# AIM-SE/AC-TSR

Hardware: AMD Instinct MI355X
Metric: user-sequences/sec fwd+bwd, AC-SASRec L=50 d=64, 1/2/4/8 MI355X (higher is better)
Workload: dtype f32; 1 GPU; ACSASRec full training step (spatial + adversarial calibrators, BASELINE configs[2]), synthetic 100000-item catalogue, B=512/GPU L=50 d=64 h=2 2 layers inner=256, CE loss, two-pass backward + Adam; global_batch=512, seq_len=50, hidden=64, heads=2, parallelism=dp1, launch=hipGraph replay per step, backward=two walks (reference protocol, trainer.py:672-686)

## Files before the change

### ac_tsr_amd/_lib.py

```python
from __future__ import annotations

import ctypes as C
import os
import subprocess

_HERE = os.path.dirname(os.path.abspath(__file__))
CSRC = os.path.join(_HERE, "csrc")
LIB_PATH = os.environ.get("ACATTN_LIB") or os.path.join(CSRC, "libacattn.so")
HEADER_PATH = os.path.join(os.path.dirname(_HERE), "include", "acattn.h")

ABI_VERSION = 34
MAX_MASKS = 8
NSTAT = 8
MASK_STRUCTURED, MASK_DENSE_LL, MASK_DENSE_L = 0, 1, 2
COMBINE = {"fixed": 0, "gate": 1, "annealing": 2}
RICH = {"none": 0, "fixed": 1, "trainable": 2}
RNG_EXPLICIT, RNG_COUNTER = 0, 1
FWD_AUTO, FWD_STREAM, FWD_STAGED, FWD_GENERAL = 0, 1, 2, 3
BWD_AUTO, BWD_STREAM, BWD_ROW = 0, 1, 2

_f = C.c_void_p


class Problem(C.Structure):
# ... 157 lines not shown
    "acattn_split_weights_many": (C.c_int, [C.POINTER(SplitLayer), C.c_int32, C.c_void_p]),
    "acattn_projections_split_bytes": (C.c_int64, [C.c_int32, C.c_int32]),
    "acattn_adam_step": (C.c_int, [C.POINTER(AdamGroup), C.c_double, C.c_double, C.c_double, C.c_double, C.c_double, _f,
                                   C.c_void_p]),
    "acattn_adam_step_cached": (C.c_int, [C.POINTER(AdamGroup), C.c_double, C.c_double, C.c_double, C.c_double, C.c_double, _f,
                                          C.c_void_p, C.c_void_p]),
    "acattn_select_adam_grid": (C.c_int, [C.c_int]),
    "acattn_dense_ce_fwd": (C.c_int, [_f, C.c_int64, C.c_int64, _f, _f, _f, C.c_void_p]),
    "acattn_dense_ce_bwd": (C.c_int, [_f, _f, _f, _f, C.c_int64, C.c_int64, _f, C.c_void_p]),
    "acattn_step_inputs": (C.c_int, [C.POINTER(C.c_void_p), C.POINTER(C.c_void_p), C.POINTER(C.c_int64), C.c_int32, C.c_void_p,
                                     C.c_void_p, C.c_void_p, C.c_int32, C.c_void_p]),
    "acattn_sum_rows": (C.c_int, [_f, _f, C.c_int32, C.c_int32, C.c_int32, C.c_void_p]),
    "acattn_sum_rows_pair": (C.c_int, [_f, _f, C.c_int32, C.c_int32, C.c_int32, _f, _f, C.c_int32, C.c_int32, C.c_int32, C.c_void_p]),
    "acattn_mask_penalty_fwd": (C.c_int, [_f, C.c_int64, _f, _f, C.c_void_p]),
    "acattn_mask_penalty_partial": (C.c_int, [_f, C.c_int64, _f, C.c_void_p]),
    "acattn_mask_penalty_partial_multi": (C.c_int, [C.c_void_p, C.c_int32, C.c_int64, _f, C.c_void_p]),
    "acattn_mask_penalty_bwd_scaled_multi": (C.c_int, [C.c_void_p, _f, _f, C.c_float, C.c_int64, C.c_void_p, C.c_int32,
                                                       C.c_void_p]),
    "acattn_attacked_loss_finish": (C.c_int, [_f, C.c_int32, _f, C.c_int32, C.c_int64, C.c_float, _f, _f, C.c_int32,
                                              C.c_void_p]),
    "acattn_mask_penalty_rows": (C.c_int, [_f, C.c_int32, C.c_int32, C.c_int32, _f, C.c_void_p]),
    "acattn_attacked_loss_finish_rows": (C.c_int, [_f, C.c_int32, C.c_void_p, C.c_int32, C.c_int32, C.c_float, _f, _f, C.c_int32,
                                                  C.c_void_p]),
    "acattn_attacked_loss_finish_rows_pair": (C.c_int, [_f, C.c_int32, C.c_void_p, C.c_int32, C.c_int32, C.c_float, _f, _f,
                                                       C.c_int32, _f, C.c_int32, _f, C.c_void_p]),
    "acattn_mask_penalty_drows": (C.c_int, [_f, _f, C.c_float, C.c_int32, C.c_void_p, C.c_int32, C.c_void_p]),
    "acattn_mask_penalty_drows_dir": (C.c_int, [_f, _f, C.c_float, C.c_int32, C.c_void_p, C.c_int32, _f, _f, C.c_int32, C.c_void_p]),
    "acattn_mask_penalty_bwd_scaled": (C.c_int, [_f, _f, _f, C.c_float, C.c_int64, _f, C.c_void_p]),
    "acattn_mask_penalty_bwd": (C.c_int, [_f, _f, _f, C.c_int64, _f, C.c_void_p]),
    "acattn_linear_wgrad_workspace_bytes": (C.c_int64, [C.c_int64, C.c_int32, C.c_int32]),
    "acattn_linear_wgrad_grouped": (C.c_int, [C.c_void_p, C.c_void_p, C.c_void_p, C.c_void_p, C.c_void_p, C.c_void_p,
                                               C.c_int32, C.c_int64, _f, C.c_void_p]),
    "acattn_linear_wgrad": (C.c_int, [_f, _f, C.c_int64, C.c_int32, C.c_int32, _f, _f, _f, C.c_void_p]),
    "acattn_linear_wgrad_grouped_partial": (C.c_int, [C.c_void_p, C.c_void_p, C.c_void_p, C.c_void_p, C.c_void_p, C.c_int32,
                                                       C.c_int64, C.c_void_p, C.c_void_p, C.c_void_p, C.c_void_p, C.c_void_p]),
    "acattn_linear_wgrad_reduce_many": (C.c_int, [C.c_void_p, C.c_void_p, C.c_void_p, C.c_void_p, C.c_void_p, C.c_void_p,
                                                   C.c_void_p, C.c_int32, C.c_void_p, C.c_void_p, C.c_void_p, C.c_void_p,
                                                   C.c_int32, C.c_void_p]),
    "acattn_select_forward_kernel": (C.c_int, [C.c_int]),
    "acattn_select_backward_kernel": (C.c_int, [C.c_int]),
    "acattn_calibrated_attention_bwd_workspace_bytes": (C.c_int64, [C.POINTER(Problem)]),
    "acattn_rng_materialize": (C.c_int, [C.c_int32, C.c_int32, C.c_int32, C.c_uint64, C.c_float, _f, _f, _f, _f,
                                         C.c_void_p]),
}

_lib = None


class AcattnError(RuntimeError):
    pass


def build(verbose: bool = False) -> str:
    jobs = str(min(8, os.cpu_count() or 1))
    res = subprocess.run(["make", "-C", CSRC, "-j", jobs], capture_output=not verbose, text=True)
    if res.returncode != 0:
        raise AcattnError("building libacattn.so failed:\n" + (res.stdout or "") + (res.stderr or ""))
    return LIB_PATH


def load() -> C.CDLL:
    global _lib
    if _lib is not None:
        return _lib
    if not os.path.exists(LIB_PATH):
        raise AcattnError(
# ... 24 lines not shown
```

### ac_tsr_amd/csrc/acattn_api.hip

```cpp
#include <stdint.h>
#include <stdio.h>
#include <string.h>

#include <algorithm>

#include "acattn_common.h"

namespace {
thread_local char g_err[256] = "";

int fail(const char* msg) {
  snprintf(g_err, sizeof(g_err), "%s", msg);
  return -1;
}

int check_problem(const acattn_problem* p) {
  if (!p) return fail("problem is NULL");
  if (p->B < 1 || p->L < 1 || p->H < 1 || p->n_heads < 1) return fail("B, L, H, n_heads must be positive");
  if (p->H % p->n_heads != 0)
    return fail("The hidden size is not a multiple of the number of attention heads");
  const int dh = p->H / p->n_heads;
  if (dh != 16 && dh != 32 && dh != 64 && dh != 128) return fail("unsupported head size: dh must be 16, 32, 64 or 128");
  if (p->L > 208) return fail("unsupported sequence length: L must be <= 208");
  if (!p->q || !p->k || !p->v) return fail("q, k, v must be non-NULL");
// ... 585 lines not shown
  if (rc > 0) snprintf(g_err, sizeof(g_err), "HIP launch failed: %s", hipGetErrorString((hipError_t)rc));
  return rc;
}

int acattn_adam_step_cached(const acattn_adam_group* g, double lr, double beta1, double beta2, double eps, double weight_decay,
                            int32_t* done, void* cache, void* stream) {
  if (!g || !done || !cache) return fail("group, done and cache must be non-NULL");
  if (((uintptr_t)cache & 15) != 0) return fail("cache must be 16-byte aligned");
  if (g->n_tensors < 1 || g->n_tensors > ACATTN_ADAM_MAX_TENSORS) return fail("1 <= n_tensors <= ACATTN_ADAM_MAX_TENSORS");
  int64_t trips = 0;
  for (int t = 0; t < g->n_tensors; ++t) {
    if (!g->param[t] || !g->grad[t] || !g->exp_avg[t] || !g->exp_avg_sq[t] || !g->step[t])
      return fail("param, grad, exp_avg, exp_avg_sq and step of every tensor must be non-NULL");
    if (g->numel[t] < 1) return fail("numel must be positive");
    trips += (g->numel[t] + 1023) / 1024;
  }
  if (trips >= (1ll << 30)) return fail("too many elements for one launch");
  if (!(beta1 >= 0 && beta1 < 1 && beta2 >= 0 && beta2 < 1)) return fail("betas must lie in [0, 1)");
  const int rc = acattn_launch_adam_step_cached(*g, lr, beta1, beta2, eps, weight_decay, done, cache, (hipStream_t)stream);
  if (rc > 0) snprintf(g_err, sizeof(g_err), "HIP launch failed: %s", hipGetErrorString((hipError_t)rc));
  return rc;
}

int acattn_select_adam_grid(int workgroups) {
  if (workgroups < 0 || workgroups > (1 << 20)) return fail("workgroups: 0 (by the device's compute units) or a positive count");
  return acattn_select_adam_grid_choice(workgroups);
}

int64_t acattn_linear_wgrad_workspace_bytes(int64_t M, int32_t K, int32_t N) {
  if (M < 1 || K < 1 || N < 1) return fail("M, K, N must be positive");
  return acattn_linear_wgrad_ws_bytes(M, K, N);
}

int acattn_linear_wgrad_grouped(const float* const* x, const float* const* dy, const int32_t* K, const int32_t* N,
                                float* const* dw, float* const* db, int32_t n_items, int64_t M, void* workspace,
                                void* stream) {
  if (!x || !dy || !K || !N || !dw || !db || !workspace) return fail("x, dy, K, N, dw, db and workspace must be non-NULL");
  if (n_items < 1 || n_items > ACATTN_WGRAD_MAX_GROUP) return fail("n_items must lie in [1, ACATTN_WGRAD_MAX_GROUP]");
  if (M < 1) return fail("M must be positive");
  for (int i = 0; i < n_items; ++i) {
    if (!x[i] || !dy[i] || !dw[i]) return fail("every item needs x, dy and dw");
    if (K[i] < 1 || N[i] < 1) return fail("K and N must be positive");
    if (M * (int64_t)std::max(K[i], N[i]) >= (1LL << 40)) return fail("matrix too large");
  }
  const int rc = acattn_launch_linear_wgrad(x, dy, (const int*)K, (const int*)N, dw, db, n_items, M, workspace,
                                            (hipStream_t)stream);
  if (rc > 0) snprintf(g_err, sizeof(g_err), "HIP launch failed: %s", hipGetErrorString((hipError_t)rc));
  return rc;
}

int acattn_linear_wgrad_grouped_partial(const float* const* x, const float* const* dy, const int32_t* K, const int32_t* N,
                                        const int32_t* want_bias, int32_t n_items, int64_t M, void* workspace, int32_t* n_partials,
                                        int64_t* w_offset, int64_t* b_offset, void* stream) {
  if (!x || !dy || !K || !N || !want_bias || !workspace || !n_partials || !w_offset || !b_offset)
    return fail("x, dy, K, N, want_bias, workspace, n_partials, w_offset and b_offset must be non-NULL");
  if (n_items < 1 || n_items > ACATTN_WGRAD_MAX_GROUP) return fail("n_items must lie in [1, ACATTN_WGRAD_MAX_GROUP]");
  if (M < 1) return fail("M must be positive");
  float* dw[ACATTN_WGRAD_MAX_GROUP];
  float* db[ACATTN_WGRAD_MAX_GROUP];
  for (int i = 0; i < n_items; ++i) {
    if (!x[i] || !dy[i]) return fail("every item needs x and dy");
    if (K[i] < 1 || N[i] < 1) return fail("K and N must be positive");
    if (M * (int64_t)std::max(K[i], N[i]) >= (1LL << 40)) return fail("matrix too large");
    dw[i] = nullptr;
    db[i] = want_bias[i] ? (float*)workspace : nullptr;
  }
  int P = 0;
  long long wo[ACATTN_WGRAD_MAX_GROUP], bo[ACATTN_WGRAD_MAX_GROUP];
  const int rc = acattn_launch_linear_wgrad(x, dy, (const int*)K, (const int*)N, dw, db, n_items, M, workspace,
                                            (hipStream_t)stream, &P, wo, bo);
  if (rc > 0) snprintf(g_err, sizeof(g_err), "HIP launch failed: %s", hipGetErrorString((hipError_t)rc));
  *n_partials = P;
  for (int i = 0; i < n_items; ++i) {
    w_offset[i] = wo[i];
    b_offset[i] = bo[i];
  }
  return rc;
}

int acattn_linear_wgrad_reduce_many(const float* const* part_w, const float* const* part_b, const int32_t* K, const int32_t* N,
                                    const int32_t* n_partials, float* const* dw, float* const* db, int32_t n_items,
// ... 28 lines not shown
```

### ac_tsr_amd/csrc/acattn_common.h

```cpp
#pragma once
#include <hip/hip_runtime.h>
#include <stdint.h>

#include <type_traits>

#include "acattn.h"

typedef float f4 __attribute__((ext_vector_type(4)));
typedef float f4u __attribute__((ext_vector_type(4), aligned(4)));

#define ACATTN_NEG_INF (-__builtin_inff())
#define ACATTN_MASK_FILL (-10000.0f)
#define ACATTN_LOG_EPS (1e-24f)

__device__ __forceinline__ float quad_sum(float x) {
  auto r = __builtin_amdgcn_permlane16_swap(__float_as_uint(x), __float_as_uint(x), false, false);
  x = __uint_as_float(r[0]) + __uint_as_float(r[1]);
  auto s = __builtin_amdgcn_permlane32_swap(__float_as_uint(x), __float_as_uint(x), false, false);
  return __uint_as_float(s[0]) + __uint_as_float(s[1]);
}

__device__ __forceinline__ float quad_max(float x) {
  auto r = __builtin_amdgcn_permlane16_swap(__float_as_uint(x), __float_as_uint(x), false, false);
  x = fmaxf(__uint_as_float(r[0]), __uint_as_float(r[1]));
// ... 245 lines not shown
int acattn_launch_ce_fwd(const acattn_ce_problem& p, void* ws, float* lse, float* row_loss, hipStream_t stream);
int acattn_launch_ce_fwd_dir(const acattn_ce_problem& p, void* ws, float* lse, float* row_loss, float* dir,
                             hipStream_t stream);
int acattn_launch_ce_bwd(const acattn_ce_problem& p, const float* lse, const float* coef, void* ws, float* d_out,
                         float* d_table, hipStream_t stream);
int acattn_launch_ln_fwd(const acattn_ln_problem& p, float* y, float* stats, hipStream_t stream);
int acattn_launch_ln_bwd(const acattn_ln_problem& p, const float* dy, const float* stats, float* dz, float* dres,
                         float* dgb_part, hipStream_t stream);
int acattn_launch_sum_rows(const float* x, float* out, int batch, int R, int C, hipStream_t stream);
int acattn_launch_sum_rows_pair(const float* x1, float* out1, int batch1, int R1, int C1, const float* x2, float* out2,
                                int batch2, int R2, int C2, hipStream_t stream);
void acattn_set_error(const char* msg);
bool acattn_proj_supported(int H, int G);
int64_t acattn_proj_bwd_ws_bytes(const acattn_proj_problem& p);
int acattn_launch_proj_fwd(const acattn_proj_problem& p, const acattn_proj_out& o, hipStream_t stream);
int64_t acattn_proj_split_bytes(int H, int G);
bool acattn_proj_qkv_supported(int H);
int acattn_launch_proj_qkv_fwd(const acattn_proj_problem& p, const acattn_proj_out& o, hipStream_t stream);
int acattn_launch_proj_bwd(const acattn_proj_problem& p, const acattn_proj_bwd_io& io, hipStream_t stream);
bool acattn_tail_supported(int H, int I);
int acattn_tail_bwd_partial_rows(int rows);
int acattn_tail_bwd_partial_rows_h(int rows, int H);
int64_t acattn_tail_bwd_ws_bytes(int H, int I);
int acattn_select_tail_nb(int nb);
int64_t acattn_tail_split_bytes(int H, int I, int rows);
int acattn_launch_tail_split(const acattn_tail_problem& p, void* planes, hipStream_t stream);
int acattn_launch_split_many(const acattn_split_layer* layers, int n_layers, hipStream_t stream);
int acattn_launch_tail_fwd(const acattn_tail_problem& p, const acattn_tail_saved& s, hipStream_t stream);
int acattn_launch_tail_bwd(const acattn_tail_problem& p, const acattn_tail_saved& s, const acattn_tail_bwd_io& io,
                           hipStream_t stream);
int64_t acattn_linear_wgrad_ws_bytes(int64_t M, int K, int N);
int acattn_launch_linear_wgrad(const float* const* x, const float* const* dy, const int* K, const int* N,
                               float* const* dw, float* const* db, int n_items, int64_t M, void* ws, hipStream_t stream,
                               int* P_out = nullptr, long long* w_off_out = nullptr, long long* b_off_out = nullptr);
int acattn_launch_linear_wgrad_reduce_many(const float* const* part_w, const float* const* part_b, const int* K, const int* N,
                                           const int* P, float* const* dw, float* const* db, int n_items,
                                           const float* const* sr_x, float* const* sr_out, const int* sr_R, const int* sr_C,
                                           int n_sr, hipStream_t stream);
int acattn_launch_embed_fwd(const acattn_embed_problem& p, float* y, float* stats, hipStream_t stream);
int acattn_launch_embed_bwd(const acattn_embed_problem& p, const float* dy, const float* stats, int64_t padding_idx,
                            float* d_table, float* d_pos_part, float* dgb_part, hipStream_t stream);
int acattn_launch_penalty_fwd(const float* m, int64_t n, float* ws, float* norm, hipStream_t stream);
int acattn_launch_penalty_partial(const float* m, int64_t n, float* part, hipStream_t stream);
void acattn_penalty_written_set(bool v);
bool acattn_penalty_written();
int acattn_launch_penalty_rows(const float* m, int B, int nh, int L, float* pen, hipStream_t stream);
int acattn_launch_attacked_loss_finish_rows(const float* row_loss, int B, const float* const* pen, int n_masks, int count,
                                            float weight, float* out, float* scale_buf, int n_scale, hipStream_t stream,
                                            const float* row_loss_c = nullptr, int B_c = 0, float* mean_c = nullptr);
int acattn_launch_penalty_drows(const float* norms, const float* d_loss, float scale, int count, float* const* d_pen,
                                int n_masks, hipStream_t stream, const float* dir = nullptr, float* d_out = nullptr, int n_dir = 0);
int acattn_launch_attacked_loss_finish(const float* row_loss, int B, const float* part, int n_masks, int64_t mask_numel,
                                       float weight, float* out, float* scale_buf, int n_scale, hipStream_t stream);
int acattn_launch_penalty_bwd_scaled(const float* m, const float* norm, const float* d_loss, float scale, int64_t n,
                                     float* d_m, hipStream_t stream);
int acattn_launch_penalty_bwd(const float* m, const float* norm, const float* d_norm, int64_t n, float* d_m,
                              hipStream_t stream);
int acattn_launch_zero(float* p, size_t n, hipStream_t stream);
int64_t acattn_ce6_rows_bytes(const acattn_ce_problem& p);
int acattn_launch_ce6_sweep(const acattn_ce_problem& p, const float* lse, const float* coef, float* slab, float* d_table,
                            float2* part, void* rows_ws, int n_wg, int n_left, bool dir, hipStream_t stream);
int acattn_launch_ce6_onehot_reduce(const acattn_ce_problem& p, const float* coef, const float* slab, int n_slabs, float* d_out,
                                    float* d_table, hipStream_t stream);
int acattn_launch_ce6_fwd_sweep(const acattn_ce_problem& p, float2* part, void* rows_ws, int n_wg, int n_left, hipStream_t stream);
int acattn_launch_ce6_pair_sweep(const acattn_ce_problem& pa, const acattn_ce_problem& pc, float* slab, float2* part_a,
                                 void* rows_a, float2* part_c, void* rows_c, int n_wg, int n_left, hipStream_t stream);
int64_t acattn_ce_pair_ws_bytes(const acattn_ce_problem& pa, const acattn_ce_problem& pc);
// ... 19 lines not shown
```

### ac_tsr_amd/csrc/acattn_linear.hip

```cpp
#include <stdlib.h>

#include <algorithm>

#include "acattn_common.h"
#include "acattn_sumrows.h"

namespace {

constexpr int kRegs = 64;

struct WgradGroup {
  const float* x[ACATTN_WGRAD_MAX_GROUP];
  const float* dy[ACATTN_WGRAD_MAX_GROUP];
  float* dw[ACATTN_WGRAD_MAX_GROUP];
  float* db[ACATTN_WGRAD_MAX_GROUP];
  int K[ACATTN_WGRAD_MAX_GROUP];
  int N[ACATTN_WGRAD_MAX_GROUP];
  long long w_off[ACATTN_WGRAD_MAX_GROUP];
  long long b_off[ACATTN_WGRAD_MAX_GROUP];
};

__device__ __forceinline__ f4 load_rows4(const float* base, int64_t row, int64_t M, int ld, int col, int ncols) {
  f4 v = {0.f, 0.f, 0.f, 0.f};
  if (row < M) {
    const float* p = base + row * ld + col;
    if (col + 3 < ncols) {
      v = *(const f4u*)p;
    } else {
#pragma unroll
      for (int e = 0; e < 4; ++e)
        if (col + e < ncols) v[e] = p[e];
    }
  }
  return v;
}

template <int UNROLL>
__global__ void __launch_bounds__(256, 2) wgrad_partial_kernel(const WgradGroup G, const int64_t M,
                                                             float* __restrict__ ws) {
  const int it = blockIdx.z;
  const int K = G.K[it], N = G.N[it];
  const int KB = (K + 63) >> 6, NB = (N + 63) >> 6;
  if ((int)blockIdx.y >= KB * NB) return;
  const float* __restrict__ x = G.x[it];
  const float* __restrict__ dy = G.dy[it];
  float* part_w = ws + G.w_off[it];
  float* part_b = G.db[it] ? ws + G.b_off[it] : nullptr;
  const int lane = threadIdx.x & 63, wave = threadIdx.x >> 6;
  const int c = lane & 15, g = lane >> 4;
  const int blk = blockIdx.y, nb = blk / KB, kb = blk - nb * KB;
  const int P = gridDim.x;
  const int ncol = nb * 64 + 4 * c, kcol = kb * 64 + 4 * c;

  f4 acc[4][4];
#pragma unroll
  for (int a = 0; a < 4; ++a)
#pragma unroll
    for (int b = 0; b < 4; ++b) acc[a][b] = f4{0.f, 0.f, 0.f, 0.f};
  f4 bsum = {0.f, 0.f, 0.f, 0.f};

  const int64_t stride = (int64_t)P * 4 * 4, batch = stride * UNROLL;
  int64_t m0 = ((int64_t)blockIdx.x * 4 + wave) * 4;
  if ((K & 63) == 0 && (N & 63) == 0) {
    auto load_batch = [&](int64_t r0, f4 (&xv)[UNROLL], f4 (&gv)[UNROLL]) {
#pragma unroll
      for (int u = 0; u < UNROLL; ++u) {
        const int64_t row = min(r0 + u * stride + g, M - 1);
// ... 16 lines not shown
      }
    };
    f4 xa[UNROLL], ga[UNROLL], xb[UNROLL], gb[UNROLL];
    load_batch(m0, xa, ga);
#pragma nounroll
    for (; m0 < M; m0 += 2 * batch) {
      load_batch(m0 + batch, xb, gb);
      __builtin_amdgcn_sched_barrier(0);
      mma_batch(m0, xa, ga);
      load_batch(m0 + 2 * batch, xa, ga);
      __builtin_amdgcn_sched_barrier(0);
      if (m0 + batch < M) mma_batch(m0 + batch, xb, gb);
    }
  } else {
    for (; m0 < M; m0 += batch) {
      f4 xv[UNROLL], gv[UNROLL];
#pragma unroll
      for (int u = 0; u < UNROLL; ++u) {
        const int64_t row = m0 + u * stride + g;
        xv[u] = load_rows4(x, row, M, K, kcol, K);
        gv[u] = load_rows4(dy, row, M, N, ncol, N);
      }
#pragma unroll
      for (int u = 0; u < UNROLL; ++u) {
        bsum += gv[u];
#pragma unroll
        for (int a = 0; a < 4; ++a)
#pragma unroll
          for (int b = 0; b < 4; ++b) acc[a][b] = mfma16(gv[u][a], xv[u][b], acc[a][b]);
      }
    }
  }

  __shared__ float red[4 * kRegs * 64];
#pragma unroll
  for (int a = 0; a < 4; ++a)
#pragma unroll
    for (int b = 0; b < 4; ++b)
#pragma unroll
      for (int r = 0; r < 4; ++r) red[(wave * kRegs + (a * 4 + b) * 4 + r) * 64 + lane] = acc[a][b][r];
  __syncthreads();
  float* pw = part_w + ((size_t)blk * P + blockIdx.x) * (kRegs * 64);
  for (int s = threadIdx.x; s < kRegs * 64; s += 256)
    pw[s] = (red[s] + red[kRegs * 64 + s]) + (red[2 * kRegs * 64 + s] + red[3 * kRegs * 64 + s]);
  if (part_b && kb == 0) {
    __syncthreads();
    *(f4*)(red + 4 * threadIdx.x) = bsum;
    __syncthreads();
    if (threadIdx.x < 64) {
      float s = 0.f;
#pragma unroll
      for (int wg = 0; wg < 16; ++wg) s += red[4 * (wg * 16 + (threadIdx.x >> 2)) + (threadIdx.x & 3)];
      part_b[((size_t)nb * P + blockIdx.x) * 64 + threadIdx.x] = s;
    }
  }
}

__global__ void __launch_bounds__(256) wgrad_reduce_kernel(const WgradGroup G, const float* __restrict__ ws,
                                                            const int P) {
  const int it = blockIdx.z;
  const int K = G.K[it], N = G.N[it];
  const int KB = (K + 63) >> 6, NB = (N + 63) >> 6;
  if ((int)blockIdx.y >= KB * NB) return;
  float* __restrict__ dw = G.dw[it];
  float* __restrict__ db = G.db[it];
  const float* part_w = ws + G.w_off[it];
  const float* part_b = ws + G.b_off[it];
  const int blk = blockIdx.y, nb = blk / KB, kb = blk - nb * KB;
  const int sl = threadIdx.x & 31, q = threadIdx.x >> 5;
  const int s = blockIdx.x * 32 + sl;
  const float* pw = part_w + (size_t)blk * P * (kRegs * 64) + s;
  constexpr size_t PS = kRegs * 64;
  float a[8];
#pragma unroll
  for (int u = 0; u < 8; ++u) a[u] = 0.f;
  int p = q;
  for (; p + 56 < P; p += 64) {
#pragma unroll
    for (int u = 0; u < 8; ++u) a[u] += pw[(size_t)(p + 8 * u) * PS];
  }
  for (; p < P; p += 8) a[0] += pw[(size_t)p * PS];
  __shared__ float red[8][32];
  red[q][sl] = ((a[0] + a[1]) + (a[2] + a[3])) + ((a[4] + a[5]) + (a[6] + a[7]));
  __syncthreads();
  if (q == 0) {
    float v = 0.f;
#pragma unroll
    for (int u = 0; u < 8; ++u) v += red[u][sl];
// ... 66 lines not shown
  __syncthreads();
  if (q == 0) {
    float v = 0.f;
#pragma unroll
    for (int u = 0; u < 8; ++u) v += red[u][sl];
    const int reg = s >> 6, lane = s & 63;
    const int tile = reg >> 2, r = reg & 3, aa = tile >> 2, bb = tile & 3, g = lane >> 4, c = lane & 15;
    const int n = nb * 64 + 4 * (4 * g + r) + aa, k = kb * 64 + 4 * c + bb;
    if (n < N && k < K) dw[(size_t)n * K + k] = v;
  }
  if (db && kb == 0 && blockIdx.x < 2) {
    __syncthreads();
    const int col = blockIdx.x * 32 + sl, nn = nb * 64 + col;
    const float* pb = part_b + (size_t)nb * P * 64 + col;
    float sb = 0.f;
    for (int t = q; t < P; t += 8) sb += pb[(size_t)t * 64];
    red[q][sl] = sb;
    __syncthreads();
    if (q == 0 && nn < N) {
      float v = 0.f;
#pragma unroll
      for (int u = 0; u < 8; ++u) v += red[u][sl];
      db[nn] = v;
    }
  }
}

int pick_partials(int64_t M, int blocks) {
  static const int forced = getenv("ACATTN_WGRAD_PARTIALS") ? atoi(getenv("ACATTN_WGRAD_PARTIALS")) : 0;
  int p = forced > 0 ? forced : std::max(64, 128 / blocks);
  return (int)std::min<int64_t>(p, std::max<int64_t>(1, M / 64));
}

}

namespace {
int64_t item_ws_floats(int K, int N, int P) {
  const int64_t KB = (K + 63) / 64, NB = (N + 63) / 64;
  return KB * NB * P * kRegs * 64 + NB * P * 64;
}
int group_partials(int64_t M, const int* K, const int* N, int n_items) {
  int blocks = 1;
  for (int i = 0; i < n_items; ++i) blocks = std::max(blocks, ((K[i] + 63) / 64) * ((N[i] + 63) / 64));
  return pick_partials(M, blocks);
}
}

int64_t acattn_linear_wgrad_ws_bytes(int64_t M, int K, int N) {
  return item_ws_floats(K, N, pick_partials(M, 1)) * (int64_t)sizeof(float);
}

int acattn_launch_linear_wgrad(const float* const* x, const float* const* dy, const int* K, const int* N,
                               float* const* dw, float* const* db, int n_items, int64_t M, void* ws, hipStream_t stream,
                               int* P_out, long long* w_off_out, long long* b_off_out) {
  WgradGroup G{};
  const int P = group_partials(M, K, N, n_items);
  int blocks = 1;
  long long off = 0;
  for (int i = 0; i < n_items; ++i) {
    G.x[i] = x[i];
    G.dy[i] = dy[i];
    G.dw[i] = dw[i];
    G.db[i] = db[i];
    G.K[i] = K[i];
    G.N[i] = N[i];
    const long long KB = (K[i] + 63) / 64, NB = (N[i] + 63) / 64;
    G.w_off[i] = off;
    G.b_off[i] = off + KB * NB * P * kRegs * 64;
    off += item_ws_floats(K[i], N[i], P);
    blocks = std::max(blocks, (int)(KB * NB));
  }
  const int64_t groups_per_wave = ((M + 3) / 4 + (int64_t)P * 4 - 1) / ((int64_t)P * 4);
  const dim3 grid(P, blocks, n_items);
  if (groups_per_wave > 4)
    hipLaunchKernelGGL((wgrad_partial_kernel<5>), grid, dim3(256), 0, stream, G, M, (float*)ws);
  else if (groups_per_wave >= 4)
    hipLaunchKernelGGL((wgrad_partial_kernel<4>), grid, dim3(256), 0, stream, G, M, (float*)ws);
  else
    hipLaunchKernelGGL((wgrad_partial_kernel<1>), grid, dim3(256), 0, stream, G, M, (float*)ws);
  int rc = (int)hipGetLastError();
  if (rc) return rc;
  if (P_out) {
    *P_out = P;
    for (int i = 0; i < n_items; ++i) {
      w_off_out[i] = G.w_off[i];
      b_off_out[i] = G.b_off[i];
    }
    return 0;
  }
  hipLaunchKernelGGL(wgrad_reduce_kernel, dim3(kRegs * 2, blocks, n_items), dim3(256), 0, stream, G, (const float*)ws, P);
  return (int)hipGetLastError();
}

int acattn_launch_linear_wgrad_reduce_many(const float* const* part_w, const float* const* part_b, const int* K, const int* N,
                                           const int* P, float* const* dw, float* const* db, int n_items,
                                           const float* const* sr_x, float* const* sr_out, const int* sr_R, const int* sr_C,
                                           int n_sr, hipStream_t stream) {
  WgradMany G{};
  G.n_w = n_items;
  int blocks = 1;
  for (int i = 0; i < n_sr; ++i) {
    G.sr[i] = make_job(sr_x[i], sr_out[i], 1, sr_R[i], sr_C[i]);
    blocks = std::max(blocks, (G.sr[i].n_wg + kRegs * 2 - 1) / (kRegs * 2));
  }
  for (int i = 0; i < n_items; ++i) {
    G.part_w[i] = part_w[i];
    G.part_b[i] = part_b[i];
    G.dw[i] = dw[i];
    G.db[i] = db[i];
    G.K[i] = K[i];
    G.N[i] = N[i];
    G.P[i] = P[i];
// ... 6 lines not shown
```

### ac_tsr_amd/ops.py

```python
from __future__ import annotations

import ctypes as C
from dataclasses import dataclass
from typing import Optional

import torch

from . import _lib, attn_launch
from .attn_launch import _ptr, _stream, spatial_attention_bwd_launch
from .state import DEFAULT as _DEFAULT_STATE
from ._lib import Problem


@dataclass
class StructuredMask:

    key_valid: torch.Tensor
    causal: bool = True

    def dense(self) -> torch.Tensor:
        valid = self.key_valid.bool()[:, None, None, :]
        if self.causal:
            L = self.key_valid.shape[-1]
            valid = torch.tril(valid.expand(-1, -1, L, -1))
# ... 361 lines not shown
    lib = _lib.load()
    ws = torch.empty(lib.acattn_linear_wgrad_workspace_bytes(M, K, N) // 4, device=x2.device, dtype=torch.float32)
    dw = torch.empty(N, K, device=x2.device, dtype=torch.float32)
    db = torch.empty(N, device=x2.device, dtype=torch.float32) if want_bias else None
    _lib.check(lib.acattn_linear_wgrad(_ptr(x2), _ptr(g2), M, K, N, _ptr(ws), _ptr(dw), _ptr(db) if want_bias else None,
                                       _stream()), "linear_wgrad")
    return dw, db


class _MaskPenalty(torch.autograd.Function):
    @staticmethod
    def forward(ctx, m):
        _need_cuda("attack mask", m)
        m = m.contiguous()
        ws = torch.empty(_lib.PENALTY_WS_FLOATS, device=m.device, dtype=torch.float32)
        norm = torch.empty((), device=m.device, dtype=torch.float32)
        _lib.check(_lib.load().acattn_mask_penalty_fwd(_ptr(m), m.numel(), _ptr(ws), _ptr(norm), _stream()), "mask_penalty_fwd")
        ctx.save_for_backward(m, norm)
        return norm

    @staticmethod
    def backward(ctx, d_norm):
        m, norm = ctx.saved_tensors
        d_m = torch.empty_like(m)
        _lib.check(_lib.load().acattn_mask_penalty_bwd(_ptr(m), _ptr(norm), _ptr(d_norm.contiguous()), m.numel(), _ptr(d_m),
                                                       _stream()), "mask_penalty_bwd")
        return d_m


def mask_penalty(attack_mask: torch.Tensor) -> torch.Tensor:
    return _MaskPenalty.apply(attack_mask)


def linear_wgrad_grouped(items, state=None):
    lib = _lib.load()
    defer = state is not None and state.deferring()
    out = [None] * len(items)
    buckets = {}
    for pos, (x, g, wb) in enumerate(items):
        assert x.is_cuda and x.dtype == torch.float32 and g.dtype == torch.float32 and x.shape[0] == g.shape[0]
        buckets.setdefault(x.shape[0], []).append((pos, x.contiguous(), g.contiguous(), wb))
    for M, members in buckets.items():
        for s0 in range(0, len(members), _lib.WGRAD_MAX_GROUP):
            chunk = members[s0:s0 + _lib.WGRAD_MAX_GROUP]
            n = len(chunk)
            dev = chunk[0][1].device
            ws_bytes = sum(lib.acattn_linear_wgrad_workspace_bytes(M, x.shape[1], g.shape[1]) for _, x, g, _ in chunk)
            ws = torch.empty(ws_bytes // 4, device=dev, dtype=torch.float32)
            dws = [torch.empty(g.shape[1], x.shape[1], device=dev, dtype=torch.float32) for _, x, g, _ in chunk]
            dbs = [torch.empty(g.shape[1], device=dev, dtype=torch.float32) if wb else None for _, _, g, wb in chunk]
            arr = lambda ptrs: (C.c_void_p * n)(*ptrs)
            ints = lambda vals: (C.c_int32 * n)(*vals)
            if defer:
                n_part = C.c_int32(0)
                w_off, b_off = (C.c_int64 * n)(), (C.c_int64 * n)()
                _lib.check(lib.acattn_linear_wgrad_grouped_partial(
                    arr([x.data_ptr() for _, x, _, _ in chunk]), arr([g.data_ptr() for _, _, g, _ in chunk]),
                    ints([x.shape[1] for _, x, _, _ in chunk]), ints([g.shape[1] for _, _, g, _ in chunk]),
                    ints([1 if wb else 0 for _, _, _, wb in chunk]), n, M, _ptr(ws), C.byref(n_part), w_off, b_off, _stream()),
                    "linear_wgrad_grouped_partial")
                base = ws.data_ptr()
                for k, ((pos, x, g, wb), gw, gb) in enumerate(zip(chunk, dws, dbs)):
                    state.defer({"part_w": base + 4 * w_off[k], "part_b": base + 4 * b_off[k], "K": x.shape[1], "N": g.shape[1],
                                 "P": n_part.value, "dw": gw.data_ptr(), "db": None if gb is None else gb.data_ptr(),
                                 "keep": (ws.untyped_storage(), gw.untyped_storage(), None if gb is None else gb.untyped_storage())})
                    out[pos] = (gw, gb)
                continue
            _lib.check(lib.acattn_linear_wgrad_grouped(
                arr([x.data_ptr() for _, x, _, _ in chunk]), arr([g.data_ptr() for _, _, g, _ in chunk]),
                ints([x.shape[1] for _, x, _, _ in chunk]), ints([g.shape[1] for _, _, g, _ in chunk]),
                arr([t.data_ptr() for t in dws]), arr([t.data_ptr() if t is not None else None for t in dbs]), n, M,
                _ptr(ws), _stream()), "linear_wgrad_grouped")
            for (pos, _, _, _), gw, gb in zip(chunk, dws, dbs):
                out[pos] = (gw, gb)
    return out
```

### include/acattn.h

```cpp
#ifndef ACATTN_H_
#define ACATTN_H_

#include <stdint.h>

#ifdef __cplusplus
extern "C" {
#endif

#define ACATTN_ABI_VERSION 34

enum {
  ACATTN_MASK_STRUCTURED = 0,
  ACATTN_MASK_DENSE_LL = 1,
  ACATTN_MASK_DENSE_L = 2
};

enum { ACATTN_COMBINE_FIXED = 0, ACATTN_COMBINE_GATE = 1, ACATTN_COMBINE_ANNEALING = 2 };

enum { ACATTN_RICH_NONE = 0, ACATTN_RICH_FIXED = 1, ACATTN_RICH_TRAINABLE = 2 };

enum {
  ACATTN_RNG_EXPLICIT = 0,
  ACATTN_RNG_COUNTER = 1
};
// ... 173 lines not shown
int acattn_attacked_loss_finish_rows(const float* row_loss, int32_t B, const float* const* pen, int32_t n_masks, int32_t count,
                                     float weight, float* out, float* scale_buf, int32_t n_scale, void* stream);
int acattn_attacked_loss_finish_rows_pair(const float* row_loss, int32_t B, const float* const* pen, int32_t n_masks,
                                          int32_t count, float weight, float* out, float* scale_buf, int32_t n_scale,
                                          const float* row_loss_c, int32_t B_c, float* mean_c, void* stream);
int acattn_mask_penalty_drows(const float* norms, const float* d_loss, float scale, int32_t count, float* const* d_pen,
                              int32_t n_masks, void* stream);
int acattn_mask_penalty_drows_dir(const float* norms, const float* d_loss, float scale, int32_t count, float* const* d_pen,
                                  int32_t n_masks, const float* direction, float* d_out, int32_t n_dir, void* stream);
#define ACATTN_MAX_MASKS 8
int acattn_mask_penalty_partial_multi(const float* const* m, int32_t n_masks, int64_t n, float* part, void* stream);
int acattn_mask_penalty_bwd_scaled_multi(const float* const* m, const float* norms, const float* d_loss, float scale, int64_t n,
                                         float* const* d_m, int32_t n_masks, void* stream);

int64_t acattn_linear_wgrad_workspace_bytes(int64_t M, int32_t K, int32_t N);
int acattn_linear_wgrad(const float* x, const float* dy, int64_t M, int32_t K, int32_t N, void* workspace, float* dw,
                        float* db, void* stream);

#define ACATTN_WGRAD_MAX_GROUP 8
int acattn_linear_wgrad_grouped(const float* const* x, const float* const* dy, const int32_t* K, const int32_t* N,
                                float* const* dw, float* const* db, int32_t n_items, int64_t M, void* workspace,
                                void* stream);

#define ACATTN_WGRAD_MAX_REDUCE 32
#define ACATTN_SUMROWS_MAX_DEFER 8
int acattn_linear_wgrad_grouped_partial(const float* const* x, const float* const* dy, const int32_t* K, const int32_t* N,
                                        const int32_t* want_bias, int32_t n_items, int64_t M, void* workspace, int32_t* n_partials,
                                        int64_t* w_offset, int64_t* b_offset, void* stream);
int acattn_linear_wgrad_reduce_many(const float* const* part_w, const float* const* part_b, const int32_t* K, const int32_t* N,
                                    const int32_t* n_partials, float* const* dw, float* const* db, int32_t n_items,
                                    const float* const* sum_x, float* const* sum_out, const int32_t* sum_R, const int32_t* sum_C,
                                    int32_t n_sums, void* stream);

typedef struct acattn_tail_problem {
  int32_t rows, H, I;
  const float* ctx;
  const float* x;
  const float* wd;
  const float* bd;
  const float* g1;
  const float* b1;
  const float* w1;
  const float* bb1;
  const float* w2;
  const float* bb2;
  const float* g2;
  const float* b2;
  float eps1, eps2;
  float p1, p2;
  const uint8_t* keep1;
  const uint8_t* keep2;
  uint64_t seed1, seed2;
  const uint64_t* seed_device;
  const int64_t* src_index;
  int32_t src_R, src_L;
  const void* split_planes;
} acattn_tail_problem;

typedef struct acattn_tail_saved {
  float* h1;
  float* st1;
  float* a;
  float* act;
  float* h3;
  float* st2;
  float* out;
// ... 150 lines not shown
```

Baseline: 519,500 user-sequences/sec.

## Flatten grouped weight-gradient grid and plan partial count across total blocks

Replaces the 3D grid (P, max_blocks, n_items) for grouped linear weight gradients with a flat 1D grid that launches only the live workgroups, mapping each workgroup to its item via prefix offsets. A new planner picks the split-M partial count from the total block count across items so the launch fills a fixed number of slots, instead of sizing by the largest item. The new kernel adds double-buffered loads and ragged and short column paths. It risks more partials to reduce and a different workspace size, and the classic path stays available behind an env var.

```diff
diff --git a/ac_tsr_amd/_lib.py b/ac_tsr_amd/_lib.py
--- a/ac_tsr_amd/_lib.py
+++ b/ac_tsr_amd/_lib.py
@@ -213,6 +213,9 @@
     "acattn_linear_wgrad_grouped": (C.c_int, [C.c_void_p, C.c_void_p, C.c_void_p, C.c_void_p, C.c_void_p, C.c_void_p,
                                                C.c_int32, C.c_int64, _f, C.c_void_p]),
     "acattn_linear_wgrad": (C.c_int, [_f, _f, C.c_int64, C.c_int32, C.c_int32, _f, _f, _f, C.c_void_p]),
+    "acattn_linear_wgrad_grouped_ex": (C.c_int, [C.c_void_p, C.c_void_p, C.c_void_p, C.c_void_p, C.c_void_p, C.c_void_p,
+                                                  C.c_int32, C.c_int64, _f, C.c_void_p, C.c_int32]),
+    "acattn_linear_wgrad_plan": (C.c_int, [C.c_int64, C.c_void_p, C.c_void_p, C.c_int32, C.c_int32, C.c_void_p, C.c_void_p]),
     "acattn_linear_wgrad_grouped_partial": (C.c_int, [C.c_void_p, C.c_void_p, C.c_void_p, C.c_void_p, C.c_void_p, C.c_int32,
                                                        C.c_int64, C.c_void_p, C.c_void_p, C.c_void_p, C.c_void_p, C.c_void_p]),
     "acattn_linear_wgrad_reduce_many": (C.c_int, [C.c_void_p, C.c_void_p, C.c_void_p, C.c_void_p, C.c_void_p, C.c_void_p,
diff --git a/ac_tsr_amd/csrc/acattn_api.hip b/ac_tsr_amd/csrc/acattn_api.hip
--- a/ac_tsr_amd/csrc/acattn_api.hip
+++ b/ac_tsr_amd/csrc/acattn_api.hip
@@ -641,21 +641,44 @@
   return acattn_linear_wgrad_ws_bytes(M, K, N);
 }
 
-int acattn_linear_wgrad_grouped(const float* const* x, const float* const* dy, const int32_t* K, const int32_t* N,
-                                float* const* dw, float* const* db, int32_t n_items, int64_t M, void* workspace,
-                                void* stream) {
+int acattn_linear_wgrad_grouped_ex(const float* const* x, const float* const* dy, const int32_t* K, const int32_t* N,
+                                   float* const* dw, float* const* db, int32_t n_items, int64_t M, void* workspace,
+                                   void* stream, int32_t force_partials) {
   if (!x || !dy || !K || !N || !dw || !db || !workspace) return fail("x, dy, K, N, dw, db and workspace must be non-NULL");
   if (n_items < 1 || n_items > ACATTN_WGRAD_MAX_GROUP) return fail("n_items must lie in [1, ACATTN_WGRAD_MAX_GROUP]");
   if (M < 1) return fail("M must be positive");
+  if (force_partials < 0) return fail("force_partials: 0 (the planner decides) or a positive count");
   for (int i = 0; i < n_items; ++i) {
     if (!x[i] || !dy[i] || !dw[i]) return fail("every item needs x, dy and dw");
     if (K[i] < 1 || N[i] < 1) return fail("K and N must be positive");
     if (M * (int64_t)std::max(K[i], N[i]) >= (1LL << 40)) return fail("matrix too large");
   }
   const int rc = acattn_launch_linear_wgrad(x, dy, (const int*)K, (const int*)N, dw, db, n_items, M, workspace,
-                                            (hipStream_t)stream);
-  if (rc > 0) snprintf(g_err, sizeof(g_err), "HIP launch failed: %s", hipGetErrorString((hipError_t)rc));
-  return rc;
+                                            (hipStream_t)stream, nullptr, nullptr, nullptr, force_partials);
+  if (rc > 0) snprintf(g_err, sizeof(g_err), "HIP launch failed: %s", hipGetErrorString((hipError_t)rc));
+  return rc;
+}
+
+int acattn_linear_wgrad_grouped(const float* const* x, const float* const* dy, const int32_t* K, const int32_t* N,
+                                float* const* dw, float* const* db, int32_t n_items, int64_t M, void* workspace,
+                                void* stream) {
+  return acattn_linear_wgrad_grouped_ex(x, dy, K, N, dw, db, n_items, M, workspace, stream, 0);
+}
+
+int acattn_linear_wgrad_plan(int64_t M, const int32_t* K, const int32_t* N, int32_t n_items, int32_t force_partials,
+                             int32_t* n_partials, int64_t* live_workgroups) {
+  if (!K || !N || !n_partials || !live_workgroups) return fail("K, N, n_partials and live_workgroups must be non-NULL");
+  if (n_items < 1 || n_items > ACATTN_WGRAD_MAX_GROUP) return fail("n_items must lie in [1, ACATTN_WGRAD_MAX_GROUP]");
+  if (M < 1) return fail("M must be positive");
+  if (force_partials < 0) return fail("force_partials: 0 (the planner decides) or a positive count");
+  for (int i = 0; i < n_items; ++i)
+    if (K[i] < 1 || N[i] < 1) return fail("K and N must be positive");
+  int P = 0;
+  long long live = 0;
+  acattn_linear_wgrad_plan_host(M, (const int*)K, (const int*)N, n_items, force_partials, &P, &live);
+  *n_partials = P;
+  *live_workgroups = live;
+  return 0;
 }
 
 int acattn_linear_wgrad_grouped_partial(const float* const* x, const float* const* dy, const int32_t* K, const int32_t* N,
diff --git a/ac_tsr_amd/csrc/acattn_common.h b/ac_tsr_amd/csrc/acattn_common.h
--- a/ac_tsr_amd/csrc/acattn_common.h
+++ b/ac_tsr_amd/csrc/acattn_common.h
@@ -301,7 +301,10 @@
 int64_t acattn_linear_wgrad_ws_bytes(int64_t M, int K, int N);
 int acattn_launch_linear_wgrad(const float* const* x, const float* const* dy, const int* K, const int* N,
                                float* const* dw, float* const* db, int n_items, int64_t M, void* ws, hipStream_t stream,
-                               int* P_out = nullptr, long long* w_off_out = nullptr, long long* b_off_out = nullptr);
+                               int* P_out = nullptr, long long* w_off_out = nullptr, long long* b_off_out = nullptr,
+                               int force_partials = 0);
+void acattn_linear_wgrad_plan_host(int64_t M, const int* K, const int* N, int n_items, int force_partials, int* P,
+                                   long long* live);
 int acattn_launch_linear_wgrad_reduce_many(const float* const* part_w, const float* const* part_b, const int* K, const int* N,
                                            const int* P, float* const* dw, float* const* db, int n_items,
                                            const float* const* sr_x, float* const* sr_out, const int* sr_R, const int* sr_C,
diff --git a/ac_tsr_amd/csrc/acattn_linear.hip b/ac_tsr_amd/csrc/acattn_linear.hip
--- a/ac_tsr_amd/csrc/acattn_linear.hip
+++ b/ac_tsr_amd/csrc/acattn_linear.hip
@@ -1,4 +1,6 @@
+#include <limits.h>
 #include <stdlib.h>
+#include <string.h>
 
 #include <algorithm>
 
@@ -33,6 +35,33 @@
     }
   }
   return v;
+}
+
+__device__ __forceinline__ void wgrad_store_partial(const f4 (&acc)[4][4], const f4 bsum, float* part_w, float* part_b,
+                                                    const int blk, const int nb, const int kb, const int P, const int p) {
+  const int lane = threadIdx.x & 63, wave = threadIdx.x >> 6;
+  __shared__ float red[4 * kRegs * 64];
+#pragma unroll
+  for (int a = 0; a < 4; ++a)
+#pragma unroll
+    for (int b = 0; b < 4; ++b)
+#pragma unroll
+      for (int r = 0; r < 4; ++r) red[(wave * kRegs + (a * 4 + b) * 4 + r) * 64 + lane] = acc[a][b][r];
+  __syncthreads();
+  float* pw = part_w + ((size_t)blk * P + p) * (kRegs * 64);
+  for (int s = threadIdx.x; s < kRegs * 64; s += 256)
+    pw[s] = (red[s] + red[kRegs * 64 + s]) + (red[2 * kRegs * 64 + s] + red[3 * kRegs * 64 + s]);
+  if (part_b && kb == 0) {
+    __syncthreads();
+    *(f4*)(red + 4 * threadIdx.x) = bsum;
+    __syncthreads();
+    if (threadIdx.x < 64) {
+      float s = 0.f;
+#pragma unroll
+      for (int wg = 0; wg < 16; ++wg) s += red[4 * (wg * 16 + (threadIdx.x >> 2)) + (threadIdx.x & 3)];
+      part_b[((size_t)nb * P + p) * 64 + threadIdx.x] = s;
+    }
+  }
 }
 
 template <int UNROLL>
@@ -115,28 +144,137 @@
     }
   }
 
-  __shared__ float red[4 * kRegs * 64];
+  wgrad_store_partial(acc, bsum, part_w, part_b, blk, nb, kb, P, blockIdx.x);
+}
+
+struct WgradFlat {
+  WgradGroup g;
+  int first[ACATTN_WGRAD_MAX_GROUP];
+};
+
+struct RaggedCols {
+  int col;
+  int shift;
+};
+__device__ __forceinline__ RaggedCols ragged_cols(int col, int ncols) {
+  if (col + 4 <= ncols) return RaggedCols{col, 0};
+  if (col < ncols) return RaggedCols{ncols - 4, col + 4 - ncols};
+  return RaggedCols{0, 4};
+}
+struct ShiftMasks {
+  unsigned m[4];
+};
+__device__ __forceinline__ ShiftMasks shift_masks(int shift) {
+  return ShiftMasks{{shift == 0 ? ~0u : 0u, shift == 1 ? ~0u : 0u, shift == 2 ? ~0u : 0u, shift == 3 ? ~0u : 0u}};
+}
+__device__ __forceinline__ f4 ragged_take(f4 v, const ShiftMasks& k) {
+  const unsigned u0 = __float_as_uint(v[0]), u1 = __float_as_uint(v[1]), u2 = __float_as_uint(v[2]), u3 = __float_as_uint(v[3]);
+  f4 r;
+  r[0] = __uint_as_float((u0 & k.m[0]) | (u1 & k.m[1]) | (u2 & k.m[2]) | (u3 & k.m[3]));
+  r[1] = __uint_as_float((u1 & k.m[0]) | (u2 & k.m[1]) | (u3 & k.m[2]));
+  r[2] = __uint_as_float((u2 & k.m[0]) | (u3 & k.m[1]));
+  r[3] = __uint_as_float(u3 & k.m[0]);
+  return r;
+}
+__device__ __forceinline__ f4 floats_inside(const float* row, int col, int ncols) {
+  f4 v = {0.f, 0.f, 0.f, 0.f};
+#pragma unroll
+  for (int e = 0; e < 4; ++e)
+    if (col + e < ncols) v[e] = row[col + e];
+  return v;
+}
+
+enum WgradLoads { kAligned, kRagged, kShort };
+
+template <int UNROLL, WgradLoads LOADS>
+__device__ __forceinline__ void wgrad_stream(const float* x, const float* dy, int64_t m0, const int64_t M, const int K, const int N, const int kcol, const int ncol,
+                                             const int g, const int64_t stride, f4 (&acc)[4][4], f4& bsum) {
+  const int64_t batch = stride * UNROLL;
+  const RaggedCols xc = LOADS == kRagged ? ragged_cols(kcol, K) : RaggedCols{kcol, 0};
+  const RaggedCols gc = LOADS == kRagged ? ragged_cols(ncol, N) : RaggedCols{ncol, 0};
+  const ShiftMasks xm = shift_masks(xc.shift), gm = shift_masks(gc.shift);
+  auto load_batch = [&](int64_t r0, f4 (&xv)[UNROLL], f4 (&gv)[UNROLL]) {
+#pragma unroll
+    for (int u = 0; u < UNROLL; ++u) {
+      const int64_t row = min(r0 + u * stride + g, M - 1);
+      if constexpr (LOADS == kAligned) {
+        xv[u] = *(const f4*)(x + row * K + kcol);
+        gv[u] = *(const f4*)(dy + row * N + ncol);
+      } else if constexpr (LOADS == kRagged) {
+        xv[u] = *(const f4u*)(x + row * K + xc.col);
+        gv[u] = *(const f4u*)(dy + row * N + gc.col);
+      } else {
+        xv[u] = floats_inside(x + row * K, kcol, K);
+        gv[u] = floats_inside(dy + row * N, ncol, N);
+      }
+    }
+  };
+  auto mma_batch = [&](int64_t r0, const f4 (&xv)[UNROLL], const f4 (&gv)[UNROLL]) {
+#pragma unroll
+    for (int u = 0; u < UNROLL; ++u) {
+      const bool row_in = r0 + u * stride + g < M;
+      f4 gq = gv[u], xq = xv[u];
+      if constexpr (LOADS == kRagged) {
+        gq = ragged_take(gq, gm);
+        xq = ragged_take(xq, xm);
+      }
+#pragma unroll
+      for (int e = 0; e < 4; ++e) gq[e] = row_in ? gq[e] : 0.f;
+      bsum += gq;
+#pragma unroll
+      for (int a = 0; a < 4; ++a)
+#pragma unroll
+        for (int b = 0; b < 4; ++b) acc[a][b] = mfma16(gq[a], xq[b], acc[a][b]);
+    }
+  };
+  f4 xa[UNROLL], ga[UNROLL], xb[UNROLL], gb[UNROLL];
+  load_batch(m0, xa, ga);
+#pragma nounroll
+  for (; m0 < M; m0 += 2 * batch) {
+    load_batch(m0 + batch, xb, gb);
+    __builtin_amdgcn_sched_barrier(0);
+    mma_batch(m0, xa, ga);
+    load_batch(m0 + 2 * batch, xa, ga);
+    __builtin_amdgcn_sched_barrier(0);
+    if (m0 + batch < M) mma_batch(m0 + batch, xb, gb);
+  }
+}
+
+template <int UNROLL>
+__global__ void __launch_bounds__(256, 2) wgrad_flat_kernel(const WgradFlat F, const int64_t M, const int P,
+                                                          float* __restrict__ ws) {
+  const int wg = blockIdx.x;
+  int it = 0;
+#pragma unroll
+  for (int i = 1; i < ACATTN_WGRAD_MAX_GROUP; ++i) it += wg >= F.first[i];
+  const int K = F.g.K[it], N = F.g.N[it];
+  const int KB = (K + 63) >> 6;
+  const float* __restrict__ x = F.g.x[it];
+  const float* __restrict__ dy = F.g.dy[it];
+  float* part_w = ws + F.g.w_off[it];
+  float* part_b = F.g.db[it] ? ws + F.g.b_off[it] : nullptr;
+  const int lane = threadIdx.x & 63, wave = threadIdx.x >> 6;
+  const int c = lane & 15, g = lane >> 4;
+  const int local = wg - F.first[it];
+  const int blk = local / P, p = local - blk * P, nb = blk / KB, kb = blk - nb * KB;
+  const int ncol = nb * 64 + 4 * c, kcol = kb * 64 + 4 * c;
+
+  f4 acc[4][4];
 #pragma unroll
   for (int a = 0; a < 4; ++a)
 #pragma unroll
-    for (int b = 0; b < 4; ++b)
-#pragma unroll
-      for (int r = 0; r < 4; ++r) red[(wave * kRegs + (a * 4 + b) * 4 + r) * 64 + lane] = acc[a][b][r];
-  __syncthreads();
-  float* pw = part_w + ((size_t)blk * P + blockIdx.x) * (kRegs * 64);
-  for (int s = threadIdx.x; s < kRegs * 64; s += 256)
-    pw[s] = (red[s] + red[kRegs * 64 + s]) + (red[2 * kRegs * 64 + s] + red[3 * kRegs * 64 + s]);
-  if (part_b && kb == 0) {
-    __syncthreads();
-    *(f4*)(red + 4 * threadIdx.x) = bsum;
-    __syncthreads();
-    if (threadIdx.x < 64) {
-      float s = 0.f;
-#pragma unroll
-      for (int wg = 0; wg < 16; ++wg) s += red[4 * (wg * 16 + (threadIdx.x >> 2)) + (threadIdx.x & 3)];
-      part_b[((size_t)nb * P + blockIdx.x) * 64 + threadIdx.x] = s;
-    }
-  }
+    for (int b = 0; b < 4; ++b) acc[a][b] = f4{0.f, 0.f, 0.f, 0.f};
+  f4 bsum = {0.f, 0.f, 0.f, 0.f};
+
+  const int64_t stride = (int64_t)P * 4 * 4;
+  const int64_t m0 = ((int64_t)p * 4 + wave) * 4;
+  if ((K & 63) == 0 && (N & 63) == 0)
+    wgrad_stream<UNROLL, kAligned>(x, dy, m0, M, K, N, kcol, ncol, g, stride, acc, bsum);
+  else if (K >= 4 && N >= 4)
+    wgrad_stream<UNROLL, kRagged>(x, dy, m0, M, K, N, kcol, ncol, g, stride, acc, bsum);
+  else
+    wgrad_stream<UNROLL, kShort>(x, dy, m0, M, K, N, kcol, ncol, g, stride, acc, bsum);
+  wgrad_store_partial(acc, bsum, part_w, part_b, blk, nb, kb, P, p);
 }
 
 __global__ void __launch_bounds__(256) wgrad_reduce_kernel(const WgradGroup G, const float* __restrict__ ws,
@@ -269,29 +407,84 @@
   return (int)std::min<int64_t>(p, std::max<int64_t>(1, M / 64));
 }
 
-}
-
-namespace {
+constexpr int kSlots = 512, kMinPartials = 32, kMaxPartials = 128;
+
+bool wgrad_classic() {
+  static const bool classic = getenv("ACATTN_WGRAD_KERNEL") && !strcmp(getenv("ACATTN_WGRAD_KERNEL"), "classic");
+  return classic;
+}
+int forced_partials() {
+  static const int forced = getenv("ACATTN_WGRAD_PARTIALS") ? atoi(getenv("ACATTN_WGRAD_PARTIALS")) : 0;
+  return forced > 0 ? forced : 0;
+}
+int max_partials(int64_t M) { return (int)std::min<int64_t>(1 << 20, std::max<int64_t>(1, M / 64)); }
+
+int plan_partials(int64_t M, int B) {
+  int p = std::min(kSlots / B, kMaxPartials);
+  if (p < kMinPartials) {
+    int best_empty = kSlots;
+    for (int q = kMinPartials; q < 2 * kMinPartials; ++q) {
+      const int empty = (kSlots - (int)(((int64_t)B * q) % kSlots)) % kSlots;
+      if (empty < best_empty) best_empty = empty, p = q;
+    }
+  }
+  return std::min(p, max_partials(M));
+}
+
+int bound_partials(int64_t M, int blocks) {
+  if (wgrad_classic()) return pick_partials(M, 1);
+  const int forced = forced_partials();
+  const int p = forced ? forced : std::max(std::min(kSlots / blocks, kMaxPartials), 2 * kMinPartials - 1);
+  return std::min(p, max_partials(M));
+}
+
 int64_t item_ws_floats(int K, int N, int P) {
   const int64_t KB = (K + 63) / 64, NB = (N + 63) / 64;
   return KB * NB * P * kRegs * 64 + NB * P * 64;
 }
-int group_partials(int64_t M, const int* K, const int* N, int n_items) {
-  int blocks = 1;
-  for (int i = 0; i < n_items; ++i) blocks = std::max(blocks, ((K[i] + 63) / 64) * ((N[i] + 63) / 64));
-  return pick_partials(M, blocks);
-}
+
+struct WgradPlan {
+  int P;
+  int max_blocks;
+  int live;
+};
+WgradPlan plan_group(int64_t M, const int* K, const int* N, int n_items, int force_partials) {
+  int total = 0, max_blocks = 1, bound = 1 << 20;
+  for (int i = 0; i < n_items; ++i) {
+    const int b = ((K[i] + 63) / 64) * ((N[i] + 63) / 64);
+    total += b;
+    max_blocks = std::max(max_blocks, b);
+    bound = std::min(bound, bound_partials(M, b));
+  }
+  int P;
+  if (force_partials > 0)
+    P = std::min(force_partials, std::min(bound, max_partials(M)));
+  else if (wgrad_classic() || forced_partials())
+    P = pick_partials(M, max_blocks);
+  else
+    P = plan_partials(M, total);
+  return WgradPlan{P, max_blocks, P * total};
+}
+
 }
 
 int64_t acattn_linear_wgrad_ws_bytes(int64_t M, int K, int N) {
-  return item_ws_floats(K, N, pick_partials(M, 1)) * (int64_t)sizeof(float);
+  return item_ws_floats(K, N, bound_partials(M, ((K + 63) / 64) * ((N + 63) / 64))) * (int64_t)sizeof(float);
+}
+
+void acattn_linear_wgrad_plan_host(int64_t M, const int* K, const int* N, int n_items, int force_partials, int* P,
+                                   long long* live) {
+  const WgradPlan plan = plan_group(M, K, N, n_items, force_partials);
+  *P = plan.P;
+  *live = plan.live;
 }
 
 int acattn_launch_linear_wgrad(const float* const* x, const float* const* dy, const int* K, const int* N,
                                float* const* dw, float* const* db, int n_items, int64_t M, void* ws, hipStream_t stream,
-                               int* P_out, long long* w_off_out, long long* b_off_out) {
+                               int* P_out, long long* w_off_out, long long* b_off_out, int force_partials) {
   WgradGroup G{};
-  const int P = group_partials(M, K, N, n_items);
+  const WgradPlan plan = plan_group(M, K, N, n_items, force_partials);
+  const int P = plan.P;
   int blocks = 1;
   long long off = 0;
   for (int i = 0; i < n_items; ++i) {
@@ -308,13 +501,30 @@
     blocks = std::max(blocks, (int)(KB * NB));
   }
   const int64_t groups_per_wave = ((M + 3) / 4 + (int64_t)P * 4 - 1) / ((int64_t)P * 4);
-  const dim3 grid(P, blocks, n_items);
-  if (groups_per_wave > 4)
-    hipLaunchKernelGGL((wgrad_partial_kernel<5>), grid, dim3(256), 0, stream, G, M, (float*)ws);
-  else if (groups_per_wave >= 4)
-    hipLaunchKernelGGL((wgrad_partial_kernel<4>), grid, dim3(256), 0, stream, G, M, (float*)ws);
-  else
-    hipLaunchKernelGGL((wgrad_partial_kernel<1>), grid, dim3(256), 0, stream, G, M, (float*)ws);
+  if (wgrad_classic()) {
+    const dim3 grid(P, blocks, n_items);
+    if (groups_per_wave > 4)
+      hipLaunchKernelGGL((wgrad_partial_kernel<5>), grid, dim3(256), 0, stream, G, M, (float*)ws);
+    else if (groups_per_wave >= 4)
+      hipLaunchKernelGGL((wgrad_partial_kernel<4>), grid, dim3(256), 0, stream, G, M, (float*)ws);
+    else
+      hipLaunchKernelGGL((wgrad_partial_kernel<1>), grid, dim3(256), 0, stream, G, M, (float*)ws);
+  } else {
+    WgradFlat F{};
+    F.g = G;
+    int first = 0;
+    for (int i = 0; i < ACATTN_WGRAD_MAX_GROUP; ++i) {
+      F.first[i] = i < n_items ? first : INT_MAX;
+      if (i < n_items) first += ((K[i] + 63) / 64) * ((N[i] + 63) / 64) * P;
+    }
+    const dim3 grid(plan.live);
+    if (groups_per_wave > 4)
+      hipLaunchKernelGGL((wgrad_flat_kernel<5>), grid, dim3(256), 0, stream, F, M, P, (float*)ws);
+    else if (groups_per_wave >= 4)
+      hipLaunchKernelGGL((wgrad_flat_kernel<4>), grid, dim3(256), 0, stream, F, M, P, (float*)ws);
+    else
+      hipLaunchKernelGGL((wgrad_flat_kernel<1>), grid, dim3(256), 0, stream, F, M, P, (float*)ws);
+  }
   int rc = (int)hipGetLastError();
   if (rc) return rc;
   if (P_out) {
diff --git a/ac_tsr_amd/ops.py b/ac_tsr_amd/ops.py
--- a/ac_tsr_amd/ops.py
+++ b/ac_tsr_amd/ops.py
@@ -417,9 +417,10 @@
     return _MaskPenalty.apply(attack_mask)
 
 
-def linear_wgrad_grouped(items, state=None):
+def linear_wgrad_grouped(items, state=None, force_partials=0):
     lib = _lib.load()
     defer = state is not None and state.deferring()
+    assert not (defer and force_partials), "the deferred form always takes the planner's partial count"
     out = [None] * len(items)
     buckets = {}
     for pos, (x, g, wb) in enumerate(items):
@@ -451,11 +452,11 @@
                                  "keep": (ws.untyped_storage(), gw.untyped_storage(), None if gb is None else gb.untyped_storage())})
                     out[pos] = (gw, gb)
                 continue
-            _lib.check(lib.acattn_linear_wgrad_grouped(
+            _lib.check(lib.acattn_linear_wgrad_grouped_ex(
                 arr([x.data_ptr() for _, x, _, _ in chunk]), arr([g.data_ptr() for _, _, g, _ in chunk]),
                 ints([x.shape[1] for _, x, _, _ in chunk]), ints([g.shape[1] for _, _, g, _ in chunk]),
                 arr([t.data_ptr() for t in dws]), arr([t.data_ptr() if t is not None else None for t in dbs]), n, M,
-                _ptr(ws), _stream()), "linear_wgrad_grouped")
+                _ptr(ws), _stream(), force_partials), "linear_wgrad_grouped")
             for (pos, _, _, _), gw, gb in zip(chunk, dws, dbs):
                 out[pos] = (gw, gb)
     return out
diff --git a/include/acattn.h b/include/acattn.h
--- a/include/acattn.h
+++ b/include/acattn.h
@@ -229,6 +229,12 @@
                                     const float* const* sum_x, float* const* sum_out, const int32_t* sum_R, const int32_t* sum_C,
                                     int32_t n_sums, void* stream);
 
+int acattn_linear_wgrad_grouped_ex(const float* const* x, const float* const* dy, const int32_t* K, const int32_t* N,
+                                   float* const* dw, float* const* db, int32_t n_items, int64_t M, void* workspace,
+                                   void* stream, int32_t force_partials);
+int acattn_linear_wgrad_plan(int64_t M, const int32_t* K, const int32_t* N, int32_t n_items, int32_t force_partials,
+                             int32_t* n_partials, int64_t* live_workgroups);
+
 typedef struct acattn_tail_problem {
   int32_t rows, H, I;
   const float* ctx;
```

New measurement: 522,300 user-sequences/sec (median of 6 runs). No clear change (+0.5%).
